# jonasBoss/ndarray-interp

Measured on AMD Instinct MI355X. Metric: interp_array Mpoints/s (queries x lanes), 1D cubic f64, higher is better.
Workload: dtype f64; 1 GPU; Target: 1D CubicSpline NotAKnot, 4096 knots x 4096 lanes f64, 10000000 queries per GPU in 4 distinct chunks of 2500000 through a 2-slot device-output ring (sorted-unique uniform knots, unsorted uniform in-range queries; output 327.7 GB per step, never copied to the host)

## Files before the change

ndarray-interp_amd/csrc/float_host.hpp:

```cpp

template <class T>
struct Queries {
  const T* a = nullptr;
  const T* b = nullptr;
  int count() const { return b ? 2 : 1; }
  Queries operator+(uint64_t off) const { return {a + off, b ? b + off : nullptr}; }
};

struct FirstFail {
  unsigned long long f0 = NO_FAIL, f1 = NO_FAIL;
  unsigned long long first() const { return std::min(f0, f1); }
  template <class T>
  static FirstFail of(const Workspace& ws, Queries<T> q) {
    return {ws.host_status->first_fail[0], q.b ? ws.host_status->first_fail[1] : NO_FAIL};
  }
};

constexpr size_t ZERO_COPY_LIMIT = 1u << 20;

template <class Plan>
struct RingRun {
  std::unique_lock<std::mutex> own;
  std::vector<void*> slots;
  uint64_t pitch = 0, chunk = 0;
  uint32_t n_slots = 0;
  uint32_t wmax = 1;
  bool narrow_first = false;
  uint32_t n_sets = 2;
  uint64_t prepped = 0;
  std::vector<Plan> plans;
  hipStream_t side = nullptr;
};

template <class T, class Impl>
struct FloatEngine {
  Impl& self() { return static_cast<Impl&>(*this); }

  ndi_status report(Queries<T> q, int q_space, FirstFail f, uint64_t index_offset, ndi_oob_info* info) {
    const int axis = f.f0 <= f.f1 ? 0 : 1;
    const unsigned long long ff = axis ? f.f1 : f.f0;
    const T* src = axis ? q.b : q.a;
    T v;
    if (q_space == NDI_MEM_DEVICE) NDI_HIP(hipMemcpy(&v, src + ff, sizeof(T), hipMemcpyDeviceToHost));
    else v = src[ff];
    const ndi_status st = self().failure_status(v);
    if (info) {
// ... 177 lines not shown
    if (out_stride < self().lanes) return fail(NDI_BAD_ARG, "out_row_stride (%llu) < lanes (%llu)",
                                               (unsigned long long)out_stride, (unsigned long long)self().lanes);
    if (nq == 0) return NDI_OK;
    if (!q_.a || q_.count() != Impl::query_arrays || !out_) return fail(NDI_BAD_ARG, "null query / output pointer");
    SpaceLease lease(self().spaces, s);
    Workspace& ws = lease.ws;
    if (self().zero_copy_fits(nq, o.q_memspace, o.out_memspace))
      return eval_small_zero_copy(s, ws, q_, nq, (T*)out_, out_stride, info);
    const Queries<T> q = stage_queries(s, ws, q_, nq, o.q_memspace);
    return eval_body(s, ws, q, q_, o.q_memspace, nq, out_, out_stride, o, info);
  }

  static constexpr bool ring_groups = false;

  template <class Plan>
  void ring_prep(hipStream_t s, Workspace& ws, Queries<T> q, uint64_t k, uint64_t cq, RingRun<Plan>& R, int path,
                 bool beside_eval) {
    Scratch& sc = ws.sc[k % R.n_sets];
    if (k >= R.n_sets) NDI_HIP(hipStreamWaitEvent(R.side, sc.eval_done, 0));
    R.plans[k % R.n_sets] = self().prep(R.side, sc, q + k * R.chunk, cq, (T*)R.slots[k % R.n_slots], R.pitch, path,
                                        beside_eval);
    NDI_HIP(hipEventRecord(sc.prep_done, R.side));
  }

  template <class Plan>
  void ring_begin(hipStream_t s, Workspace& ws, Queries<T> q, uint64_t nq, const ndi_ring_desc* ring, uint64_t stride,
                  const ndi_eval_opts& o, RingRun<Plan>& R) {
    R.n_slots = ring->n_slots;
    R.chunk = ring->chunk_queries;
    R.slots.resize(ring->n_slots);
    R.pitch = stride;
    if (ring->slots) {
      for (uint32_t i = 0; i < ring->n_slots; ++i) R.slots[i] = ring->slots[i];
    } else {
      OwnedRing& ring_own = self().ring_own;
      R.own = std::unique_lock<std::mutex>(ring_own.mu);
      ring_own.ensure(ring->n_slots, ring->chunk_queries, stride * sizeof(T));
      for (uint32_t i = 0; i < ring->n_slots; ++i) R.slots[i] = (char*)ring_own.buf.p + (size_t)i * stride * sizeof(T);
      R.pitch = (uint64_t)ring->n_slots * stride;
    }
    R.side = ring_overlap() ? ws.side_stream() : s;
    const int mode = Impl::ring_groups ? ring_group_mode() : 0;
    R.wmax = mode ? std::min<uint32_t>({R.n_slots, (uint32_t)RING_GROUP_MAX, Workspace::MAX_SETS / 2}) : 1u;
    R.narrow_first = mode == 2;
    R.n_sets = 2 * R.wmax;
    R.plans.assign(R.n_sets, Plan{});
    for (uint32_t i = 0; i < R.n_sets; ++i) ws.sc[i].ensure_events();
    NDI_HIP(hipEventRecord(ws.order_event(), s));
    NDI_HIP(hipStreamWaitEvent(R.side, ws.order_event(), 0));
    uint64_t first = 1;
    if constexpr (Impl::ring_groups)
      if (!R.narrow_first) first = std::min<uint64_t>(R.wmax, (nq + R.chunk - 1) / R.chunk);
    for (R.prepped = 0; R.prepped < first;) {
      const uint64_t k = R.prepped++;
      ring_prep(s, ws, q, k, std::min<uint64_t>(R.chunk, nq - k * R.chunk), R, o.path, false);
      if constexpr (Impl::ring_groups)
        if (!self().groupable(R.plans[k])) break;
    }
  }

  template <class Plan>
  void ring_produce(hipStream_t s, Workspace& ws, Queries<T> q, uint64_t limit, RingRun<Plan>& R,
                    ndi_ring_consumer consume, void* user, const ndi_eval_opts& o, uint64_t q_offset, uint32_t shard) {
    std::vector<hipEvent_t> busy(R.n_slots, nullptr);
    const uint64_t nchunks = (limit + R.chunk - 1) / R.chunk;
    auto count = [&](uint64_t k) { return std::min<uint64_t>(R.chunk, limit - k * R.chunk); };
    bool solo = R.wmax == 1;
    uint64_t prepped = R.prepped;
    for (uint64_t k = 0; k < nchunks;) {
      uint32_t want = solo || (R.narrow_first && k == 0) ? 1u : (uint32_t)std::min<uint64_t>(R.wmax, nchunks - k);
      uint32_t w = 0;
      while (w < want) {
        if (k + w >= prepped) {
          ring_prep(s, ws, q, k + w, count(k + w), R, o.path, R.side != s);
          prepped = k + w + 1;
        }
        bool joins = w == 0;
        if constexpr (Impl::ring_groups) joins = joins || (self().groupable(R.plans[k % R.n_sets]) &&
                                                          self().groupable(R.plans[(k + w) % R.n_sets]));
        if (!joins) break;
        ++w;
      }
      Scratch* sets[RING_GROUP_MAX];
      Plan plans[RING_GROUP_MAX];
      for (uint32_t i = 0; i < w; ++i) {
        sets[i] = &ws.sc[(k + i) % R.n_sets];
        plans[i] = R.plans[(k + i) % R.n_sets];
        NDI_HIP(hipStreamWaitEvent(s, sets[i]->prep_done, 0));
        const uint32_t slot = (uint32_t)((k + i) % R.n_slots);
// ... 9 lines not shown
          grouped = true;
        }
      if (!grouped) self().launch_eval(s, *sets[0], plans[0]);
      for (uint32_t i = 0; i < w; ++i) NDI_HIP(hipEventRecord(sets[i]->eval_done, s));
      for (uint32_t i = 0; i < w && consume; ++i) {
        const uint32_t slot = (uint32_t)((k + i) % R.n_slots);
        ndi_ring_chunk c{};
        c.index = k + i; c.q_begin = q_offset + (k + i) * R.chunk; c.q_count = count(k + i); c.out = R.slots[slot];
        c.row_stride = R.pitch; c.slot = slot; c.shard = shard; c.stream = (void*)s;
        busy[slot] = (hipEvent_t)consume(user, &c);
        if (busy[slot]) solo = true;
      }
      k += w;
    }
    NDI_HIP(hipStreamSynchronize(s));
    NDI_HIP(hipStreamSynchronize(R.side));
    for (hipEvent_t e : busy)
      if (e) NDI_HIP(hipEventSynchronize(e));
    ws.pending = false;
  }

  ndi_status run_ring(const char* range, Queries<T> q_, uint64_t nq, const ndi_ring_desc* ring, ndi_ring_consumer consume,
                      void* user, const ndi_eval_opts* opts, ndi_oob_info* info) {
    DeviceGuard dg(self().device);
    ndi_eval_opts o{};
    if (const ndi_status vs__ = take_opts(opts, o); vs__ != NDI_OK) return vs__;
    hipStream_t s = (hipStream_t)o.stream;
    uint64_t stride = 0;
    ndi_status rs = check_ring_desc(ring, self().lanes, &stride);
    if (rs != NDI_OK) return rs;
    if (nq == 0) return NDI_OK;
    if (!q_.a || q_.count() != Impl::query_arrays) return fail(NDI_BAD_ARG, "null query pointer");
    Range rg(range);
    SpaceLease lease(self().spaces, s);
    Workspace& ws = lease.ws;
    const Queries<T> q = stage_queries(s, ws, q_, nq, o.q_memspace);
    enqueue_prepass(s, ws, q, nq);
    RingRun<typename Impl::Plan> R;
    ring_begin(s, ws, q, nq, ring, stride, o, R);
    NDI_HIP(hipStreamSynchronize(s));
    const FirstFail f = FirstFail::of(ws, q);
    const uint64_t limit = f.first() == NO_FAIL ? nq : std::min<uint64_t>(nq, f.first());
    ring_produce(s, ws, q, limit, R, consume, user, o, 0, 0);
    if (f.first() == NO_FAIL) return NDI_OK;
    return report(q_, o.q_memspace, f, 0, info);
  }

  void trim_front() {
    self().spaces.trim();
    if constexpr (Impl::ring) {
      std::lock_guard<std::mutex> g(self().ring_own.mu);
// ... 5 lines not shown
```

ndarray-interp_amd/csrc/interp1d_host.hpp:

```cpp
#pragma once

template <class A, class = void>
struct takes_knots : std::false_type {};
template <class A>
struct takes_knots<A, std::void_t<decltype(std::declval<A&>().knots)>> : std::true_type {};
template <class A, class T>
static void table_args(A& F, const Interp1DImpl<T>& h) {
  if constexpr (takes_knots<A>::value) F.knots = h.pyr.view.lv0;
  else F.pyr = h.pyr.view;
  F.data = h.data.template as<T>();
  F.ca = h.ca.template as<T>();
  F.cb = h.cb.template as<T>();
}

template <class A, class T>
static void batch_args(A& F, const Interp1DImpl<T>& h, StatusBlock* st, const T* q, T* out, uint64_t nq, uint64_t out_stride) {
  F.q = q;
  F.out = out;
  F.nq = nq;
  F.out_stride = out_stride;
  F.lanes = (uint32_t)h.lanes;
  F.mode = h.mode;
  F.first_fail = &st->first_fail[0];
}
// ... 103 lines not shown
  const size_t w_plain = best_tb(false, tb_plain);
  const size_t w_lut = (P.nq >= 4096 && h.pyr.lut_bytes != 0) ? best_tb(true, tb_lut) : 0;
  if (w_plain == 0 && w_lut == 0) return false;
  P.f_lut = w_lut != 0 && 2 * w_lut >= w_plain;
  tb_auto = P.f_lut ? tb_lut : tb_plain;
  return true;
}

template <class T>
static void fused_table_form1(const Interp1DImpl<T>& h, Plan1<T>& P, const ShortKnobs& K, unsigned tb_auto) {
  const uint64_t lanes = h.lanes;
  P.f_tlds = 0;
  P.f_tb = fused_tb_or(K, tb_auto);
  if (K.lds == 0) return;
  size_t best_waves = 0;
  const bool yk_ok = h.strategy == NDI_CUBIC_SPLINE && h.ck.p;
  const int pinned = (K.lds == 2 && !yk_ok) ? 1 : K.lds;
  for (int form : {1, 2}) {
    if (form == 2 && !yk_ok) continue;
    if (pinned > 0 && pinned <= 2 && pinned != form) continue;
    for (unsigned tb : {1024u, 512u, 256u}) {
      if (K.tb && (unsigned)K.tb != tb) continue;
      const size_t need = h.fused_lds_bytes(P.f_lut, tb, form);
      if (need > FUSED_LDS_LIMIT) continue;
      const size_t waves = wgs_per_cu(need, tb) * (tb / 64);
      if (waves > best_waves) {
        best_waves = waves;
        P.f_tlds = form;
        P.f_tb = tb;
      }
    }
// ... 221 lines not shown
}

template <class T>
static Eval1Args<T> eval1_args(const Interp1DImpl<T>& h, Scratch& sc, const Plan1<T>& P) {
  Eval1Args<T> A{};
  table_args(A, h);
  A.q = P.q;
  A.idx = sc.idx.as<uint32_t>();
  A.t = sc.t.as<T>();
  A.out = P.out;
  A.lanes = h.lanes;
  A.out_stride = P.out_stride;
  A.nq = P.nq;
  A.status = sc.status.as<StatusBlock>();
  A.n_int = (uint32_t)(h.n - 1);
#ifdef NDI_BOUNDS
  if (env_int("NDI_BOUNDS_SELFTEST", 0)) A.n_int = 1;
#endif
  return A;
}

template <bool GROUP, class T, class Args>
static void launch_bucketed(Interp1DImpl<T>& h, hipStream_t s, uint64_t LV, unsigned gx, const Args& A) {
  constexpr int CQ = Interp1DImpl<T>::BUCKETED_CQ;
  const int U = LV >= 2048 ? 8 : (LV >= 1024 ? 4 : (LV >= 512 ? 2 : 1));
  const uint64_t segs = (LV + (uint64_t)BLOCK * U - 1) / ((uint64_t)BLOCK * U);
  const dim3 grid(gx, (unsigned)std::min<uint64_t>(segs, 64));
  const bool full = LV % ((uint64_t)BLOCK * U) == 0;
  pick<ST_CUBIC, ST_LINEAR>(h.strat(), [&](auto st_) {
    constexpr int ST = st_;
    pick_or<1, 8, 4, 2>(U, [&](auto u_) {
      constexpr int UU = u_;
      pick_bool(full, [&](auto full_) {
        if constexpr (GROUP) launch1<T>(s, PC_EVAL, grid, dim3(BLOCK), 0, eval_bucketed_group_kernel<T, ST, UU, CQ, true, full_>, A);
        else launch1<T>(s, PC_EVAL, grid, dim3(BLOCK), 0, eval_bucketed_kernel<T, ST, UU, CQ, true, full_>, A);
      });
    });
  });
}

template <class T>
static void launch_bucketed1(Interp1DImpl<T>& h, hipStream_t s, Scratch& sc, const Plan1<T>& P) {
  Eval1Args<T> A = eval1_args(h, sc, P);
  A.rec = sc.perm.as<uint4>();
// ... 109 lines not shown
template <class T>
void Interp1DImpl<T>::launch_eval_group(hipStream_t s, Scratch* const* sc, const Plan* P, uint32_t w) {
  if (trace_plan())
    std::fprintf(stderr, "[ndi plan] ring bucketed L=%llu lv=%llu width=%u nq=%llu\n", (unsigned long long)lanes,
                 (unsigned long long)P[0].LV, w, (unsigned long long)P[0].nq);
  if (w == 1) {
    launch_eval(s, *sc[0], P[0]);
    return;
  }
  if (w > (uint32_t)RING_GROUP_MAX) throw HipFailure{hipErrorInvalidValue, "launch_eval_group: group too wide", __LINE__};
  EvalGroupArgs<T> G{};
  table_args(G.A, *this);
  G.A.lanes = lanes;
  G.A.out_stride = P[0].out_stride;
  G.A.n_int = (uint32_t)(n - 1);
  G.width = w;
  constexpr int CQ = BUCKETED_CQ;
  uint64_t nmax = 0;
  for (uint32_t i = 0; i < w; ++i) {
    if (!groupable(P[i]) || P[i].out_stride != P[0].out_stride || P[i].LV != P[0].LV)
      throw HipFailure{hipErrorInvalidValue, "launch_eval_group: plans of one group differ", __LINE__};
    G.rec[i] = sc[i]->perm.as<uint4>();
    G.nq[i] = P[i].nq;
    G.out[i] = P[i].out;
    G.status[i] = sc[i]->status.as<StatusBlock>();
    nmax = std::max<uint64_t>(nmax, (P[i].nq + CQ - 1) / CQ);
  }
  const uint64_t per_xcd = (nmax * w + 7) / 8;
  launch_bucketed<true>(*this, s, P[0].LV, (unsigned)std::max<uint64_t>(8, std::min<uint64_t>(per_xcd * 8, 65528)), G);
}
// ... 1 lines not shown
```

ndarray-interp_amd/csrc/kernels.hpp:

```cpp
#pragma once
#include <hip/hip_runtime.h>
#include <stdint.h>

#include <type_traits>

namespace ndi {

constexpr unsigned long long NO_FAIL = ~0ull;
constexpr int BLOCK = 256;

enum ExtrapMode : int { EX_NO = 0, EX_YES = 1, EX_PERIODIC = 2 };
enum Strat : int { ST_LINEAR = 0, ST_CUBIC = 1 };

struct StatusBlock {
  unsigned long long first_fail[2];
  unsigned long long n_valid;
  unsigned long long periodic_mismatch;
  unsigned int ticket;
  unsigned int reserved;
};

#ifdef NDI_BOUNDS
__device__ unsigned long long g_ndi_bounds[4];
__device__ __forceinline__ unsigned long long ndi_bounds_fail(int code, int line, unsigned long long idx,
                                                              unsigned long long lim) {
  if (atomicAdd(&g_ndi_bounds[0], 1ull) == 0ull) {
    g_ndi_bounds[1] = ((unsigned long long)code << 32) | (unsigned)line;
// ... 622 lines not shown
template <class T>
struct Eval1Args {
  const T* knots;
  const T* data;
  const T* ca;
  const T* cb;
  const T* q;
  const uint32_t* idx;
  const T* t;
  T* out;
  uint64_t lanes, out_stride, nq;
  const StatusBlock* status;
  const uint4* rec;
  uint32_t run;
  uint32_t n_int;
};

template <class T>
__device__ __forceinline__ uint4 make_rec(uint32_t qi, uint32_t i, T s);
template <>
__device__ __forceinline__ uint4 make_rec<double>(uint32_t qi, uint32_t i, double s) {
  const unsigned long long b = __builtin_bit_cast(unsigned long long, s);
  return make_uint4(qi, i, (uint32_t)b, (uint32_t)(b >> 32));
}
template <>
__device__ __forceinline__ uint4 make_rec<float>(uint32_t qi, uint32_t i, float s) {
  return make_uint4(qi, i, __builtin_bit_cast(uint32_t, s), 0u);
}
__device__ __forceinline__ double rec_value(const uint4& r, double) {
  return __builtin_bit_cast(double, ((unsigned long long)r.w << 32) | r.z);
// ... 18 lines not shown
    c.c0 = x2 - x1;
    c.c1 = xq - x1;
    c.c2 = T(0);
  }
  return c;
}

template <class T, int STRAT, class V>
__device__ __forceinline__ V row_point(const RowCoef<T, STRAT>& c, V yl, V yr, V a, V b) {
  if (STRAT == ST_CUBIC) {
    return c.c0 * yl + c.c1 * yr + c.c2 * (a * c.c0 + b * c.c1);
  } else {
    V m = (yr - yl) / c.c0;
    return m * c.c1 + yl;
  }
}

template <bool NT, class V>
__device__ __forceinline__ void store_stream(V* p, V v) {
  if (NT) __builtin_nontemporal_store(v, p);
  else *p = v;
}

constexpr int SMALL_LANES = 16;

template <class T>
struct EvalSmallArgs {
  Pyramid<T> pyr;
  const T* data;
  const T* ca;
// ... 1223 lines not shown
  for (uint32_t i = threadIdx.x; i < nb; i += BLOCK) cur[i] = off[i] + base[i];
  __syncthreads();
  const uint64_t q_begin = (uint64_t)blockIdx.x * slice;
  uint64_t q_end = q_begin + slice;
  if (q_end > nq) q_end = nq;
  for (uint64_t qi = q_begin + threadIdx.x; qi < q_end; qi += BLOCK) {
    const uint32_t i = NDI_CHK(idx[qi], nb, BC_BIN);
    const uint32_t pos = NDI_CHK(atomicAdd(&cur[i], 1u), nq, BC_POSITION);
    rec[pos] = make_rec<T>((uint32_t)qi, i, sval[qi]);
  }
}

template <class T, int STRAT, int U, int CQ, bool NT = true, bool FULL = false>
__global__ __launch_bounds__(BLOCK) void eval_bucketed_kernel(Eval1Args<T> A) {
  constexpr int VN = Wide<T>::N;
  using V = typename VecT<T, VN>::type;
  __shared__ uint32_t s_q[CQ];
  __shared__ uint32_t s_i[CQ];
  __shared__ T s_s[CQ];
  const uint64_t LV = A.lanes / VN;
  const uint32_t seg_vecs = BLOCK * U;
  const uint32_t segs = (uint32_t)((LV + seg_vecs - 1) / seg_vecs);
  const unsigned long long n_valid = A.nq;
  unsigned long long limit = A.status->first_fail[0];
  if (limit > A.nq) limit = A.nq;
  const uint64_t nchunks = (n_valid + CQ - 1) / CQ;
  const uint64_t per = (nchunks + 7) / 8;
  const uint64_t run = A.run ? A.run : 1;
  const uint64_t runs_per_xcd = (per + run - 1) / run;
  for (uint32_t seg = blockIdx.y; seg < segs; seg += gridDim.y) {
// ... 6 lines not shown
      if (c_end > nchunks) c_end = nchunks;
      V ryl[U], ryr[U], ra[U], rb[U];
      uint32_t cur = 0xffffffffu;
      for (uint64_t chunk = c_begin; chunk < c_end; ++chunk) {
        const uint64_t p0 = chunk * CQ;
        const uint32_t cnt = (n_valid - p0 < (uint64_t)CQ) ? (uint32_t)(n_valid - p0) : (uint32_t)CQ;
        __syncthreads();
        for (uint32_t j = threadIdx.x; j < cnt; j += BLOCK) {
          const uint4 r = A.rec[p0 + j];
          s_q[j] = r.x;
          s_i[j] = r.y;
          s_s[j] = rec_value(r, T(0));
        }
        __syncthreads();
        auto emit = [&](uint32_t i, uint32_t qi, T sj) {
          const RowCoef<T, STRAT> c = row_coef<T, STRAT>(A.knots, i, sj, sj);
          V* o = reinterpret_cast<V*>(A.out + (uint64_t)qi * A.out_stride);
#pragma unroll
          for (int u = 0; u < U; ++u) {
            const uint64_t v = v0 + (uint64_t)u * BLOCK;
            if (FULL || v < LV) store_stream<NT>(o + v, row_point<T, STRAT, V>(c, ryl[u], ryr[u], ra[u], rb[u]));
          }
        };
        for (uint32_t j = 0; j < cnt;) {
          const uint32_t i = NDI_CHK((uint32_t)__builtin_amdgcn_readfirstlane((int)s_i[j]), A.n_int, BC_INTERVAL);
          const uint32_t qi = NDI_CHK((uint32_t)__builtin_amdgcn_readfirstlane((int)s_q[j]), A.nq, BC_QUERY);
          if (qi >= limit) { ++j; continue; }
          if (i != cur) {
            cur = i;
            const V* yl = reinterpret_cast<const V*>(A.data + (uint64_t)i * A.lanes);
            const V* yr = yl + LV;
            const V* pa = reinterpret_cast<const V*>(A.ca + (uint64_t)i * A.lanes);
            const V* pb = reinterpret_cast<const V*>(A.cb + (uint64_t)i * A.lanes);
#pragma unroll
            for (int u = 0; u < U; ++u) {
              const uint64_t v = v0 + (uint64_t)u * BLOCK;
              if (FULL || v < LV) {
                ryl[u] = yl[v];
                ryr[u] = yr[v];
                if (STRAT == ST_CUBIC) {
                  ra[u] = pa[v];
                  rb[u] = pb[v];
                }
              }
            }
          }
          emit(i, qi, s_s[j]);
          ++j;
        }
      }
    }
  }
}

constexpr int RING_GROUP_MAX = 4;
template <class T>
struct EvalGroupArgs {
  Eval1Args<T> A;
  const uint4* rec[RING_GROUP_MAX];
  uint64_t nq[RING_GROUP_MAX];
  T* out[RING_GROUP_MAX];
  const StatusBlock* status[RING_GROUP_MAX];
  uint32_t width;
};

template <class T, int STRAT, int U, int CQ, bool NT = true, bool FULL = false>
__global__ __launch_bounds__(BLOCK) void eval_bucketed_group_kernel(EvalGroupArgs<T> G) {
  constexpr int VN = Wide<T>::N;
  using V = typename VecT<T, VN>::type;
  __shared__ uint32_t s_q[CQ];
  __shared__ uint32_t s_i[CQ];
  __shared__ T s_s[CQ];
  const Eval1Args<T>& A = G.A;
  const uint64_t LV = A.lanes / VN;
  const uint32_t seg_vecs = BLOCK * U;
  const uint32_t segs = (uint32_t)((LV + seg_vecs - 1) / seg_vecs);
  const uint32_t width = G.width;
  uint64_t nmax = 0;
#pragma unroll
  for (int w = 0; w < RING_GROUP_MAX; ++w) {
    const uint64_t n_w = (uint32_t)w < width ? (G.nq[w] + CQ - 1) / CQ : 0;
    if (n_w > nmax) nmax = n_w;
  }
// ... 29 lines not shown
      unsigned long long limit = status->first_fail[0];
      if (limit > nq) limit = nq;
      V ryl[U], ryr[U], ra[U], rb[U];
      uint32_t cur = 0xffffffffu;
      const uint64_t p0 = chunk * CQ;
      const uint32_t cnt = (n_valid - p0 < (uint64_t)CQ) ? (uint32_t)(n_valid - p0) : (uint32_t)CQ;
      __syncthreads();
      for (uint32_t j = threadIdx.x; j < cnt; j += BLOCK) {
        const uint4 r = rec[p0 + j];
        s_q[j] = r.x;
        s_i[j] = r.y;
        s_s[j] = rec_value(r, T(0));
      }
      __syncthreads();
      auto emit = [&](uint32_t i, uint32_t qi, T sj) {
        const RowCoef<T, STRAT> cf = row_coef<T, STRAT>(A.knots, i, sj, sj);
        V* o = reinterpret_cast<V*>(out + (uint64_t)qi * A.out_stride);
#pragma unroll
        for (int u = 0; u < U; ++u) {
          const uint64_t v = v0 + (uint64_t)u * BLOCK;
          if (FULL || v < LV) store_stream<NT>(o + v, row_point<T, STRAT, V>(cf, ryl[u], ryr[u], ra[u], rb[u]));
        }
      };
      for (uint32_t j = 0; j < cnt;) {
        const uint32_t i = NDI_CHK((uint32_t)__builtin_amdgcn_readfirstlane((int)s_i[j]), A.n_int, BC_INTERVAL);
        const uint32_t qi = NDI_CHK((uint32_t)__builtin_amdgcn_readfirstlane((int)s_q[j]), nq, BC_QUERY);
        if (qi >= limit) { ++j; continue; }
        if (i != cur) {
          cur = i;
          const V* yl = reinterpret_cast<const V*>(A.data + (uint64_t)i * A.lanes);
          const V* yr = yl + LV;
          const V* pa = reinterpret_cast<const V*>(A.ca + (uint64_t)i * A.lanes);
          const V* pb = reinterpret_cast<const V*>(A.cb + (uint64_t)i * A.lanes);
#pragma unroll
          for (int u = 0; u < U; ++u) {
            const uint64_t v = v0 + (uint64_t)u * BLOCK;
            if (FULL || v < LV) {
              ryl[u] = yl[v];
              ryr[u] = yr[v];
              if (STRAT == ST_CUBIC) {
                ra[u] = pa[v];
                rb[u] = pb[v];
              }
            }
          }
        }
        emit(i, qi, s_s[j]);
        ++j;
      }
    }
  }
}

template <class T, int STRAT, int G, int CQ, bool NT = true>
__global__ __launch_bounds__(BLOCK) void eval_bucketed_short_kernel(Eval1Args<T> A) {
  constexpr int VN = Wide<T>::N;
  using V = typename VecT<T, VN>::type;
// ... 1885 lines not shown
      if (b < cnt) {
        const uint64_t i = hi - 1 - b;
        const T k = (ri[b] - upc[b] * k_next) / midc[b];
        const T dy = y_hi - yl[b];
        sa[i * L] = k * dxc[b] - dy;
        sb[i * L] = dy - k_next * dxc[b];
        if (KOUT) A.kout[i * L + l] = k;
        k_next = k;
        y_hi = yl[b];
      }
    }
    hi -= (uint64_t)cnt;
  }
}

template <class T, int RW>
__global__ __launch_bounds__(256) void spline_build_wide_kernel(BuildArgs<T> A) {
  extern __shared__ __attribute__((aligned(16))) unsigned char smem_raw[];
  constexpr int RB = 3 * RW;
  T* const s_r = reinterpret_cast<T*>(smem_raw);
  T* const s_y = s_r + 2 * RB * 64;
  T* const s_f = s_y + 2 * RB * 64;
  const uint32_t tid = threadIdx.x, lane = tid & 63u;
  const uint32_t wave = __builtin_amdgcn_readfirstlane(tid >> 6);
  const uint64_t n = A.n, L = A.lanes;
  const uint64_t l0 = (uint64_t)blockIdx.x * 64u, l = l0 + lane;
  const bool live = l < L;
  const uint64_t lc = live ? l : L - 1u;
  const T* __restrict__ const y = A.data;
  T* const sa = A.ca;
  T* const sb = A.cb;
// ... 92 lines not shown
      const uint64_t i = b < hi ? hi - 1 - b : 0;
      T* const f = s_f + (size_t)buf * 4 * RB;
      const SharedDivisor<T> sd = shared_divisor<T>(A.midp[i]);
      f[0 * RB + b] = A.up[i];
      f[1 * RB + b] = sd.d;
      f[2 * RB + b] = sd.ok ? sd.r : T(0);
      f[3 * RB + b] = A.dx[i];
    }
  };
  T k_next = T(0), y_hi = T(0);
  if (wave == 0) {
    const T rhs_last = spline_rhs_at<T, false, false>(A, n - 1, lc);
    const T r_last = rhs_last - A.w[n - 1] * r_prev;
    k_next = r_last / A.midp[n - 1];
    y_hi = y[(n - 1) * L + lc];
  } else {
    produce_bwd(0u, n - 1);
  }
  __syncthreads();
  auto back_row = [&](uint64_t i, T ri, T yl, T up, T mid, T rmid, T dxi) {
    SharedDivisor<T> sd;
    sd.d = mid; sd.r = rmid; sd.ok = rmid > T(0);
    const T num = ri - up * k_next;
    bool ok;
    T k = div_shared_fast<T>(num, sd, ok);
    if (__builtin_expect(!ok, 0)) k = num / mid;
    const T dy = y_hi - yl;
    if (live) {
      sa[i * L + l] = k * dxi - dy;
      sb[i * L + l] = dy - k_next * dxi;
    }
    k_next = k;
    y_hi = yl;
  };
  for (uint64_t blk = 0; blk < bblk; ++blk) {
    const uint64_t hi = n - 1 - blk * RB;
    const uint32_t buf = (uint32_t)(blk & 1u);
    if (wave != 0) {
      if (blk + 1 < bblk) produce_bwd(buf ^ 1u, hi - RB);
    } else {
      const T* const r = s_r + (size_t)buf * RB * 64;
      const T* const yy = s_y + (size_t)buf * RB * 64;
      const T* const f = s_f + (size_t)buf * 4 * RB;
      if (hi >= (uint64_t)RB) {
#pragma unroll
// ... 426 lines not shown
```

ndarray-interp_amd/csrc/ndinterp_api.hip:

```cpp
#include <dlfcn.h>

#include <algorithm>
#include <atomic>
#include <chrono>
#include <condition_variable>
#include <cmath>
#include <cstdlib>
#include <cstring>
#include <functional>
#include <limits>
#include <map>
#include <memory>
#include <mutex>
#include <set>
#include <shared_mutex>
#include <stdexcept>
#include <thread>
#include <unordered_map>
#include <utility>
#include <vector>

#include "common.hpp"
#include "host_logic.hpp"
#include "kernels.hpp"
// ... 411 lines not shown
  }
  void ensure_events() {
    if (!prep_done) NDI_HIP(hipEventCreateWithFlags(&prep_done, hipEventDisableTiming));
    if (!eval_done) NDI_HIP(hipEventCreateWithFlags(&eval_done, hipEventDisableTiming));
  }
};

struct Workspace {
  static constexpr uint32_t MAX_SETS = 8;
  Scratch sc[MAX_SETS];
  DevBuf status, qdev, qdev2, stage;
  StatusBlock* host_status = nullptr;
  void* pin = nullptr;
  void* pin_dev = nullptr;
  size_t pin_bytes = 0;
  hipStream_t side = nullptr;
  hipEvent_t ev = nullptr;
  uint64_t last_nq = 0;
  const void* last_q = nullptr;
  const void* last_q2 = nullptr;
  int last_q_space = NDI_MEM_DEVICE;
  bool pending = false;
  int users = 0;
  uint64_t last_use = 0;
  ~Workspace() {
    if (side) (void)hipStreamDestroy(side);
    if (ev) (void)hipEventDestroy(ev);
    if (host_status) (void)hipHostFree(host_status);
    if (pin) (void)hipHostFree(pin);
  }
  void ensure_pin(size_t need) {
    if (need <= pin_bytes) return;
    if (pin) (void)hipHostFree(pin);
    pin = nullptr;
    pin_dev = nullptr;
    pin_bytes = 0;
    NDI_HIP(hipHostMalloc(&pin, need, hipHostMallocMapped | hipHostMallocPortable));
    NDI_HIP(hipHostGetDevicePointer(&pin_dev, pin, 0));
    pin_bytes = need;
  }
  template <class U>
  U* pin_device(const void* host_ptr) const {
    return reinterpret_cast<U*>((char*)pin_dev + ((const char*)host_ptr - (const char*)pin));
  }
  void ensure_status() {
    status.reserve(sizeof(StatusBlock));
    for (int i = 0; i < 2; ++i) sc[i].status.reserve(sizeof(StatusBlock));
    if (!host_status) NDI_HIP(hipHostMalloc((void**)&host_status, sizeof(StatusBlock), hipHostMallocDefault));
  }
  hipStream_t side_stream() {
    if (!side) {
      int lo = 0, hi = 0;
      NDI_HIP(hipDeviceGetStreamPriorityRange(&lo, &hi));
      NDI_HIP(hipStreamCreateWithPriority(&side, hipStreamNonBlocking, hi));
    }
    return side;
  }
  hipEvent_t order_event() {
    if (!ev) NDI_HIP(hipEventCreateWithFlags(&ev, hipEventDisableTiming));
    return ev;
  }
};

struct SpaceSet {
  static constexpr size_t MAX_IDLE = 16;
  std::mutex mu;
  std::map<SpaceKey, std::unique_ptr<Workspace>> map;
  uint64_t tick = 0;

  Workspace& acquire(hipStream_t s) {
    std::lock_guard<std::mutex> g(mu);
// ... 418 lines not shown
      packed_state.store(1, std::memory_order_release);
      return true;
    }
    (void)hipGetLastError();
    if (s != packed_stream) NDI_HIP(hipStreamWaitEvent(s, packed_ev, 0));
    return true;
  }

  void adopt_arena(bool cubic, bool with_k) {
    auto al = [](size_t b) { return (b + 255) & ~(size_t)255; };
    uint64_t block = 1;
    while ((uint64_t)64 * block < n) block *= 2;
    const size_t pyr_b = al((n + (n + block - 1) / block) * sizeof(T));
    const size_t data_b = al((size_t)n * lanes * sizeof(T));
    const size_t tab_b = cubic ? al((size_t)(n - 1) * lanes * sizeof(T)) : 0;
    const size_t k_b = (cubic && with_k && 2 * data_b <= FUSED_LDS_LIMIT) ? data_b : 0;
    const size_t total = pyr_b + data_b + 2 * tab_b + k_b;
    if (total > ((size_t)1 << 20)) return;
    arena.reserve(total);
    char* p0 = static_cast<char*>(arena.p);
    pyr.buf.adopt(p0, pyr_b);
    data.adopt(p0 + pyr_b, data_b);
    if (tab_b) {
      ca.adopt(p0 + pyr_b + data_b, tab_b);
      cb.adopt(p0 + pyr_b + data_b + tab_b, tab_b);
    }
    if (k_b) ck.adopt(p0 + pyr_b + data_b + 2 * tab_b, k_b);
  }

  uint64_t signature() const override {
    uint64_t h = fnv1a(FNV_SEED, pyr.host_knots.data(), pyr.host_knots.size() * sizeof(T));
    const uint64_t f[3] = {n, (uint64_t)strategy | ((uint64_t)rule << 8) | ((uint64_t)deriv << 16), (uint64_t)mode};
    return fnv1a(h, f, sizeof(f));
  }

  T* reserve_k() {
    static const Knob keep{"NDI_SPLINE_KEEP_K", 1, Knob::live};
    if (!keep.get() || lanes > 2048 || fused_lds_bytes(false, 256, 2) > FUSED_LDS_LIMIT) {
      ck.release();
      return nullptr;
    }
    ck.reserve((size_t)n * lanes * sizeof(T));
    return ck.as<T>();
  }

  ndi_status build_spline(const ndi_interp1d_desc& d);
  ndi_status build_hermite(const void* dydx, int memspace);

  using Plan = Plan1<T>;
  Plan prep(hipStream_t s, Scratch& sc, const T* q, uint64_t nq, T* out, uint64_t out_stride, int path,
            bool beside_eval = false, int flags = 0);
  void launch_eval(hipStream_t s, Scratch& sc, const Plan& P);

// ... 1054 lines not shown
  uint64_t lo, cnt;
  DeviceGuard dg;
  hipStream_t s;
  SpaceLease lease;
  Workspace& ws;
  Queries<T> q_src, q;
  uint64_t stride = 0;
  RingRun<typename Impl::Plan> R;
  Shard(const Job<Impl>& j, uint32_t i_, uint32_t n)
      : J(j), i(i_), h(j.H[i_]), lo(shard_lo(j.nq, i_, n)), cnt(shard_lo(j.nq, i_ + 1, n) - shard_lo(j.nq, i_, n)),
        dg(h->device), s((hipStream_t)(j.io ? j.io[i_].stream : nullptr)), lease(h->spaces, s), ws(lease.ws),
        q_src(j.q_src(i_, n)) {}
  void pre(unsigned long long* fx, unsigned long long* fy) {
    if (!cnt) return;
    q = h->stage_queries(s, ws, q_src, cnt, J.o.q_memspace);
    h->enqueue_prepass(s, ws, q, cnt);
    if (J.rings) {
      (void)check_ring_desc(&J.rings[i], h->lanes, &stride);
      h->ring_begin(s, ws, q, cnt, &J.rings[i], stride, J.o, R);
    }
    NDI_HIP(hipStreamSynchronize(s));
    const FirstFail f = FirstFail::of(ws, q);
    *fx = f.f0;
    *fy = f.f1;
  }
  ndi_status run(uint64_t limit) {
    if (!cnt) return NDI_OK;
    if (J.rings) {
      h->ring_produce(s, ws, q, limit, R, J.consume, J.user, J.o, lo, i);
      return NDI_OK;
// ... 1102 lines not shown
```

ndarray-interp_amd/csrc/spline_build_host.hpp:

```cpp
#pragma once

template <class T>
static void reserve_tables(Interp1DImpl<T>& h) {
  const size_t tab = (size_t)(h.n - 1) * h.lanes * sizeof(T);
  h.ca.reserve(tab);
  h.cb.reserve(tab);
}

static unsigned build_rows_grid(uint64_t n, uint64_t lanes) {
  return (unsigned)std::max<uint64_t>(1, std::min<uint64_t>((n * lanes + BLOCK - 1) / BLOCK, 65536));
}
static unsigned build_lane_grid(uint64_t lanes) { return (unsigned)((lanes + 63) / 64); }

template <class T>
static BuildArgs<T> build_args(Interp1DImpl<T>& h, const SplinePlan<T>& P) {
  BuildArgs<T> A{};
  A.data = h.data.template as<T>();
  A.ca = h.ca.template as<T>();
  A.cb = h.cb.template as<T>();
  A.n = h.n;
  A.lanes = h.lanes;
  A.left_kind = P.left_kind;
  A.right_kind = P.right_kind;
  A.left_val = P.left_val;
// ... 183 lines not shown
  }
  NDI_HIP(hipGetLastError());
  if (per) NDI_HIP(hipMemcpy(&hs, tmp.p, sizeof(hs), hipMemcpyDeviceToHost));
  else NDI_HIP(hipStreamSynchronize(s));
}

template <class T>
static void build_serial(int spline_mode, const BuildArgs<T>& A, const BuildTemp<T>& tmp, StatusBlock& hs) {
  const uint64_t n = A.n, lanes = A.lanes;
  const unsigned grid = build_lane_grid(lanes);
  hipStream_t s = nullptr;
  switch (spline_mode) {
    case SPLINE_GENERAL: {
      static const Knob wide_knob{"NDI_SPLINE_WIDE", -1, Knob::live};
      const int wide_env = wide_knob.get();
      if (!A.kout && n >= 4 && (wide_env > 0 || (wide_env < 0 && lanes >= 1024))) {
        constexpr int RW = 16, RBW = 3 * RW;
        const size_t shm = (size_t)(4 * RBW * 64 + 2 * 4 * RBW) * sizeof(T);
        auto kern = spline_build_wide_kernel<T, RW>;
        allow_dynamic_lds(reinterpret_cast<const void*>(kern), (int)shm);
        hipLaunchKernelGGL(kern, dim3(grid), dim3(256), shm, s, A);
        break;
      }
      hipLaunchKernelGGL((spline_rhs_kernel<T, false>), dim3(build_rows_grid(n, lanes)), dim3(BLOCK), 0, s, A);
      launch_build_general<T, false, false>(A);
      break;
    }
    case SPLINE_PARABOLA3:
      hipLaunchKernelGGL(spline_build_n3_kernel<T>, dim3(grid), dim3(64), 0, s, A, 0);
      break;
    case SPLINE_PERIODIC3:
      hipLaunchKernelGGL(spline_build_n3_kernel<T>, dim3(grid), dim3(64), 0, s, A, 1);
      break;
    case SPLINE_PERIODIC:
      hipLaunchKernelGGL(spline_build_periodic_kernel<T>, dim3(grid), dim3(64), 0, s, A);
      break;
// ... 154 lines not shown
```

Before: 863,200 Mpoints/s.

## Use knot-slope table in bucketed cubic eval and split ring prep across side streams

```diff
diff --git a/ndarray-interp_amd/csrc/float_host.hpp b/ndarray-interp_amd/csrc/float_host.hpp
--- a/ndarray-interp_amd/csrc/float_host.hpp
+++ b/ndarray-interp_amd/csrc/float_host.hpp
@@ -30,6 +30,8 @@
   uint64_t prepped = 0;
   std::vector<Plan> plans;
   hipStream_t side = nullptr;
+  hipStream_t sides[Workspace::MAX_SIDES] = {};
+  uint32_t n_sides = 1;
 };
 
 template <class T, class Impl>
@@ -237,14 +239,16 @@
   static constexpr bool ring_groups = false;
 
   template <class Plan>
-  void ring_prep(hipStream_t s, Workspace& ws, Queries<T> q, uint64_t k, uint64_t cq, RingRun<Plan>& R, int path,
+  void ring_prep(hipStream_t side, Workspace& ws, Queries<T> q, uint64_t k, uint64_t cq, RingRun<Plan>& R, int path,
                  bool beside_eval) {
     Scratch& sc = ws.sc[k % R.n_sets];
-    if (k >= R.n_sets) NDI_HIP(hipStreamWaitEvent(R.side, sc.eval_done, 0));
-    R.plans[k % R.n_sets] = self().prep(R.side, sc, q + k * R.chunk, cq, (T*)R.slots[k % R.n_slots], R.pitch, path,
+    if (k >= R.n_sets) NDI_HIP(hipStreamWaitEvent(side, sc.eval_done, 0));
+    R.plans[k % R.n_sets] = self().prep(side, sc, q + k * R.chunk, cq, (T*)R.slots[k % R.n_slots], R.pitch, path,
                                         beside_eval);
-    NDI_HIP(hipEventRecord(sc.prep_done, R.side));
-  }
+    NDI_HIP(hipEventRecord(sc.prep_done, side));
+  }
+
+  void ring_order(hipStream_t s, Workspace& ws) { NDI_HIP(hipEventRecord(ws.order_event(), s)); }
 
   template <class Plan>
   void ring_begin(hipStream_t s, Workspace& ws, Queries<T> q, uint64_t nq, const ndi_ring_desc* ring, uint64_t stride,
@@ -262,21 +266,27 @@
       for (uint32_t i = 0; i < ring->n_slots; ++i) R.slots[i] = (char*)ring_own.buf.p + (size_t)i * stride * sizeof(T);
       R.pitch = (uint64_t)ring->n_slots * stride;
     }
-    R.side = ring_overlap() ? ws.side_stream() : s;
+    R.side = R.sides[0] = ring_overlap() ? ws.side_stream(0) : s;
+    R.n_sides = 1;
     const int mode = Impl::ring_groups ? ring_group_mode() : 0;
     R.wmax = mode ? std::min<uint32_t>({R.n_slots, (uint32_t)RING_GROUP_MAX, Workspace::MAX_SETS / 2}) : 1u;
     R.narrow_first = mode == 2;
     R.n_sets = 2 * R.wmax;
     R.plans.assign(R.n_sets, Plan{});
     for (uint32_t i = 0; i < R.n_sets; ++i) ws.sc[i].ensure_events();
-    NDI_HIP(hipEventRecord(ws.order_event(), s));
-    NDI_HIP(hipStreamWaitEvent(R.side, ws.order_event(), 0));
     uint64_t first = 1;
     if constexpr (Impl::ring_groups)
       if (!R.narrow_first) first = std::min<uint64_t>(R.wmax, (nq + R.chunk - 1) / R.chunk);
+    if (ring_overlap())
+      while (R.n_sides < std::min<uint64_t>(first, Workspace::MAX_SIDES)) {
+        R.sides[R.n_sides] = ws.side_stream(R.n_sides);
+        ++R.n_sides;
+      }
+    for (uint32_t j = 0; j < R.n_sides; ++j)
+      if (R.sides[j] != s) NDI_HIP(hipStreamWaitEvent(R.sides[j], ws.order_event(), 0));
     for (R.prepped = 0; R.prepped < first;) {
       const uint64_t k = R.prepped++;
-      ring_prep(s, ws, q, k, std::min<uint64_t>(R.chunk, nq - k * R.chunk), R, o.path, false);
+      ring_prep(R.sides[k % R.n_sides], ws, q, k, std::min<uint64_t>(R.chunk, nq - k * R.chunk), R, o.path, false);
       if constexpr (Impl::ring_groups)
         if (!self().groupable(R.plans[k])) break;
     }
@@ -295,7 +305,7 @@
       uint32_t w = 0;
       while (w < want) {
         if (k + w >= prepped) {
-          ring_prep(s, ws, q, k + w, count(k + w), R, o.path, R.side != s);
+          ring_prep(R.side, ws, q, k + w, count(k + w), R, o.path, R.side != s);
           prepped = k + w + 1;
         }
         bool joins = w == 0;
@@ -335,7 +345,7 @@
       k += w;
     }
     NDI_HIP(hipStreamSynchronize(s));
-    NDI_HIP(hipStreamSynchronize(R.side));
+    for (uint32_t j = 0; j < R.n_sides; ++j) NDI_HIP(hipStreamSynchronize(R.sides[j]));
     for (hipEvent_t e : busy)
       if (e) NDI_HIP(hipEventSynchronize(e));
     ws.pending = false;
@@ -356,6 +366,7 @@
     SpaceLease lease(self().spaces, s);
     Workspace& ws = lease.ws;
     const Queries<T> q = stage_queries(s, ws, q_, nq, o.q_memspace);
+    ring_order(s, ws);
     enqueue_prepass(s, ws, q, nq);
     RingRun<typename Impl::Plan> R;
     ring_begin(s, ws, q, nq, ring, stride, o, R);
diff --git a/ndarray-interp_amd/csrc/interp1d_host.hpp b/ndarray-interp_amd/csrc/interp1d_host.hpp
--- a/ndarray-interp_amd/csrc/interp1d_host.hpp
+++ b/ndarray-interp_amd/csrc/interp1d_host.hpp
@@ -141,7 +141,7 @@
   P.f_tb = fused_tb_or(K, tb_auto);
   if (K.lds == 0) return;
   size_t best_waves = 0;
-  const bool yk_ok = h.strategy == NDI_CUBIC_SPLINE && h.ck.p;
+  const bool yk_ok = h.strategy == NDI_CUBIC_SPLINE && h.ck.p && h.k_fits_lds();
   const int pinned = (K.lds == 2 && !yk_ok) ? 1 : K.lds;
   for (int form : {1, 2}) {
     if (form == 2 && !yk_ok) continue;
@@ -393,11 +393,15 @@
   A.nq = P.nq;
   A.status = sc.status.as<StatusBlock>();
   A.n_int = (uint32_t)(h.n - 1);
+  A.ck = h.ck.template as<T>();
 #ifdef NDI_BOUNDS
   if (env_int("NDI_BOUNDS_SELFTEST", 0)) A.n_int = 1;
 #endif
   return A;
 }
+
+template <class T>
+static bool bucketed_k_rows(const Interp1DImpl<T>& h) { return h.ck.p != nullptr && h.k_for_long_rows(); }
 
 template <bool GROUP, class T, class Args>
 static void launch_bucketed(Interp1DImpl<T>& h, hipStream_t s, uint64_t LV, unsigned gx, const Args& A) {
@@ -406,7 +410,9 @@
   const uint64_t segs = (LV + (uint64_t)BLOCK * U - 1) / ((uint64_t)BLOCK * U);
   const dim3 grid(gx, (unsigned)std::min<uint64_t>(segs, 64));
   const bool full = LV % ((uint64_t)BLOCK * U) == 0;
-  pick<ST_CUBIC, ST_LINEAR>(h.strat(), [&](auto st_) {
+  if (trace_plan() && h.strategy == NDI_CUBIC_SPLINE)
+    std::fprintf(stderr, "[ndi rows] bucketed tables=%s u=%d full=%d\n", bucketed_k_rows(h) ? "{y,k}" : "{y,a,b}", U, (int)full);
+  pick<ST_CUBIC, ST_LINEAR, ST_CUBIC_K>(bucketed_k_rows(h) ? (int)ST_CUBIC_K : h.strat(), [&](auto st_) {
     constexpr int ST = st_;
     pick_or<1, 8, 4, 2>(U, [&](auto u_) {
       constexpr int UU = u_;
@@ -546,6 +552,7 @@
   G.A.lanes = lanes;
   G.A.out_stride = P[0].out_stride;
   G.A.n_int = (uint32_t)(n - 1);
+  G.A.ck = ck.template as<T>();
   G.width = w;
   constexpr int CQ = BUCKETED_CQ;
   uint64_t nmax = 0;
diff --git a/ndarray-interp_amd/csrc/kernels.hpp b/ndarray-interp_amd/csrc/kernels.hpp
--- a/ndarray-interp_amd/csrc/kernels.hpp
+++ b/ndarray-interp_amd/csrc/kernels.hpp
@@ -10,7 +10,8 @@
 constexpr int BLOCK = 256;
 
 enum ExtrapMode : int { EX_NO = 0, EX_YES = 1, EX_PERIODIC = 2 };
-enum Strat : int { ST_LINEAR = 0, ST_CUBIC = 1 };
+enum Strat : int { ST_LINEAR = 0, ST_CUBIC = 1, ST_CUBIC_K = 2 };
+constexpr int poly_strat(int strat) { return strat == ST_CUBIC_K ? (int)ST_CUBIC : strat; }
 
 struct StatusBlock {
   unsigned long long first_fail[2];
@@ -663,6 +664,7 @@
   const uint4* rec;
   uint32_t run;
   uint32_t n_int;
+  const T* ck;
 };
 
 template <class T>
@@ -711,6 +713,19 @@
     V m = (yr - yl) / c.c0;
     return m * c.c1 + yl;
   }
+}
+
+constexpr int vmcnt_imm(int n) { return (n & 15) | ((n >> 4) << 14) | (7 << 4) | (15 << 8); }
+__device__ __forceinline__ void wait_vmcnt(int n) {
+#define NDI_VMCNT(N) case N: __builtin_amdgcn_s_waitcnt(vmcnt_imm(N)); break;
+  switch (n) {
+    NDI_VMCNT(0) NDI_VMCNT(1) NDI_VMCNT(2) NDI_VMCNT(3) NDI_VMCNT(4) NDI_VMCNT(5) NDI_VMCNT(6) NDI_VMCNT(7)
+    NDI_VMCNT(8) NDI_VMCNT(9) NDI_VMCNT(10) NDI_VMCNT(11) NDI_VMCNT(12) NDI_VMCNT(13) NDI_VMCNT(14) NDI_VMCNT(15)
+    NDI_VMCNT(16) NDI_VMCNT(17) NDI_VMCNT(18) NDI_VMCNT(19) NDI_VMCNT(20) NDI_VMCNT(21) NDI_VMCNT(22) NDI_VMCNT(23)
+    NDI_VMCNT(24) NDI_VMCNT(25) NDI_VMCNT(26) NDI_VMCNT(27) NDI_VMCNT(28) NDI_VMCNT(29) NDI_VMCNT(30) NDI_VMCNT(31)
+    default: break;
+  }
+#undef NDI_VMCNT
 }
 
 template <bool NT, class V>
@@ -1964,6 +1979,7 @@
 template <class T, int STRAT, int U, int CQ, bool NT = true, bool FULL = false>
 __global__ __launch_bounds__(BLOCK) void eval_bucketed_kernel(Eval1Args<T> A) {
   constexpr int VN = Wide<T>::N;
+  constexpr int PS = poly_strat(STRAT);
   using V = typename VecT<T, VN>::type;
   __shared__ uint32_t s_q[CQ];
   __shared__ uint32_t s_i[CQ];
@@ -2000,12 +2016,13 @@
         }
         __syncthreads();
         auto emit = [&](uint32_t i, uint32_t qi, T sj) {
-          const RowCoef<T, STRAT> c = row_coef<T, STRAT>(A.knots, i, sj, sj);
+          const RowCoef<T, PS> c = row_coef<T, PS>(A.knots, i, sj, sj);
           V* o = reinterpret_cast<V*>(A.out + (uint64_t)qi * A.out_stride);
 #pragma unroll
           for (int u = 0; u < U; ++u) {
             const uint64_t v = v0 + (uint64_t)u * BLOCK;
-            if (FULL || v < LV) store_stream<NT>(o + v, row_point<T, STRAT, V>(c, ryl[u], ryr[u], ra[u], rb[u]));
+            if (STRAT == ST_CUBIC_K) wait_vmcnt(4 * U - 4 - 3 * u);
+            if (FULL || v < LV) store_stream<NT>(o + v, row_point<T, PS, V>(c, ryl[u], ryr[u], ra[u], rb[u]));
           }
         };
         for (uint32_t j = 0; j < cnt;) {
@@ -2016,17 +2033,29 @@
             cur = i;
             const V* yl = reinterpret_cast<const V*>(A.data + (uint64_t)i * A.lanes);
             const V* yr = yl + LV;
-            const V* pa = reinterpret_cast<const V*>(A.ca + (uint64_t)i * A.lanes);
-            const V* pb = reinterpret_cast<const V*>(A.cb + (uint64_t)i * A.lanes);
+            const V* pa = reinterpret_cast<const V*>((STRAT == ST_CUBIC_K ? A.ck : A.ca) + (uint64_t)i * A.lanes);
+            const V* pb = STRAT == ST_CUBIC_K ? pa + LV : reinterpret_cast<const V*>(A.cb + (uint64_t)i * A.lanes);
 #pragma unroll
             for (int u = 0; u < U; ++u) {
               const uint64_t v = v0 + (uint64_t)u * BLOCK;
               if (FULL || v < LV) {
                 ryl[u] = yl[v];
                 ryr[u] = yr[v];
-                if (STRAT == ST_CUBIC) {
+                if (STRAT != ST_LINEAR) {
                   ra[u] = pa[v];
                   rb[u] = pb[v];
+                }
+              }
+            }
+            if (STRAT == ST_CUBIC_K) {
+              const T dx = A.knots[i + 1] - A.knots[i];
+#pragma unroll
+              for (int u = 0; u < U; ++u) {
+                const uint64_t v = v0 + (uint64_t)u * BLOCK;
+                if (FULL || v < LV) {
+                  const V dy = ryr[u] - ryl[u];
+                  ra[u] = ra[u] * dx - dy;
+                  rb[u] = dy - rb[u] * dx;
                 }
               }
             }
@@ -2053,6 +2082,7 @@
 template <class T, int STRAT, int U, int CQ, bool NT = true, bool FULL = false>
 __global__ __launch_bounds__(BLOCK) void eval_bucketed_group_kernel(EvalGroupArgs<T> G) {
   constexpr int VN = Wide<T>::N;
+  constexpr int PS = poly_strat(STRAT);
   using V = typename VecT<T, VN>::type;
   __shared__ uint32_t s_q[CQ];
   __shared__ uint32_t s_i[CQ];
@@ -2112,12 +2142,13 @@
       }
       __syncthreads();
       auto emit = [&](uint32_t i, uint32_t qi, T sj) {
-        const RowCoef<T, STRAT> cf = row_coef<T, STRAT>(A.knots, i, sj, sj);
+        const RowCoef<T, PS> cf = row_coef<T, PS>(A.knots, i, sj, sj);
         V* o = reinterpret_cast<V*>(out + (uint64_t)qi * A.out_stride);
 #pragma unroll
         for (int u = 0; u < U; ++u) {
           const uint64_t v = v0 + (uint64_t)u * BLOCK;
-          if (FULL || v < LV) store_stream<NT>(o + v, row_point<T, STRAT, V>(cf, ryl[u], ryr[u], ra[u], rb[u]));
+          if (STRAT == ST_CUBIC_K) wait_vmcnt(4 * U - 4 - 3 * u);
+          if (FULL || v < LV) store_stream<NT>(o + v, row_point<T, PS, V>(cf, ryl[u], ryr[u], ra[u], rb[u]));
         }
       };
       for (uint32_t j = 0; j < cnt;) {
@@ -2128,17 +2159,29 @@
           cur = i;
           const V* yl = reinterpret_cast<const V*>(A.data + (uint64_t)i * A.lanes);
           const V* yr = yl + LV;
-          const V* pa = reinterpret_cast<const V*>(A.ca + (uint64_t)i * A.lanes);
-          const V* pb = reinterpret_cast<const V*>(A.cb + (uint64_t)i * A.lanes);
+          const V* pa = reinterpret_cast<const V*>((STRAT == ST_CUBIC_K ? A.ck : A.ca) + (uint64_t)i * A.lanes);
+          const V* pb = STRAT == ST_CUBIC_K ? pa + LV : reinterpret_cast<const V*>(A.cb + (uint64_t)i * A.lanes);
 #pragma unroll
           for (int u = 0; u < U; ++u) {
             const uint64_t v = v0 + (uint64_t)u * BLOCK;
             if (FULL || v < LV) {
               ryl[u] = yl[v];
               ryr[u] = yr[v];
-              if (STRAT == ST_CUBIC) {
+              if (STRAT != ST_LINEAR) {
                 ra[u] = pa[v];
                 rb[u] = pb[v];
+              }
+            }
+          }
+          if (STRAT == ST_CUBIC_K) {
+            const T dx = A.knots[i + 1] - A.knots[i];
+#pragma unroll
+            for (int u = 0; u < U; ++u) {
+              const uint64_t v = v0 + (uint64_t)u * BLOCK;
+              if (FULL || v < LV) {
+                const V dy = ryr[u] - ryl[u];
+                ra[u] = ra[u] * dx - dy;
+                rb[u] = dy - rb[u] * dx;
               }
             }
           }
@@ -4054,7 +4097,7 @@
   }
 }
 
-template <class T, int RW>
+template <class T, int RW, bool KOUT = false>
 __global__ __launch_bounds__(256) void spline_build_wide_kernel(BuildArgs<T> A) {
   extern __shared__ __attribute__((aligned(16))) unsigned char smem_raw[];
   constexpr int RB = 3 * RW;
@@ -4177,6 +4220,7 @@
     const T r_last = rhs_last - A.w[n - 1] * r_prev;
     k_next = r_last / A.midp[n - 1];
     y_hi = y[(n - 1) * L + lc];
+    if (KOUT && live) A.kout[(n - 1) * L + l] = k_next;
   } else {
     produce_bwd(0u, n - 1);
   }
@@ -4192,6 +4236,7 @@
     if (live) {
       sa[i * L + l] = k * dxi - dy;
       sb[i * L + l] = dy - k_next * dxi;
+      if (KOUT) A.kout[i * L + l] = k;
     }
     k_next = k;
     y_hi = yl;
diff --git a/ndarray-interp_amd/csrc/ndinterp_api.hip b/ndarray-interp_amd/csrc/ndinterp_api.hip
--- a/ndarray-interp_amd/csrc/ndinterp_api.hip
+++ b/ndarray-interp_amd/csrc/ndinterp_api.hip
@@ -449,7 +449,8 @@
   void* pin = nullptr;
   void* pin_dev = nullptr;
   size_t pin_bytes = 0;
-  hipStream_t side = nullptr;
+  static constexpr uint32_t MAX_SIDES = 2;
+  hipStream_t side[MAX_SIDES] = {};
   hipEvent_t ev = nullptr;
   uint64_t last_nq = 0;
   const void* last_q = nullptr;
@@ -459,7 +460,8 @@
   int users = 0;
   uint64_t last_use = 0;
   ~Workspace() {
-    if (side) (void)hipStreamDestroy(side);
+    for (hipStream_t sd : side)
+      if (sd) (void)hipStreamDestroy(sd);
     if (ev) (void)hipEventDestroy(ev);
     if (host_status) (void)hipHostFree(host_status);
     if (pin) (void)hipHostFree(pin);
@@ -483,13 +485,13 @@
     for (int i = 0; i < 2; ++i) sc[i].status.reserve(sizeof(StatusBlock));
     if (!host_status) NDI_HIP(hipHostMalloc((void**)&host_status, sizeof(StatusBlock), hipHostMallocDefault));
   }
-  hipStream_t side_stream() {
-    if (!side) {
+  hipStream_t side_stream(uint32_t j) {
+    if (!side[j]) {
       int lo = 0, hi = 0;
       NDI_HIP(hipDeviceGetStreamPriorityRange(&lo, &hi));
-      NDI_HIP(hipStreamCreateWithPriority(&side, hipStreamNonBlocking, hi));
-    }
-    return side;
+      NDI_HIP(hipStreamCreateWithPriority(&side[j], hipStreamNonBlocking, hi));
+    }
+    return side[j];
   }
   hipEvent_t order_event() {
     if (!ev) NDI_HIP(hipEventCreateWithFlags(&ev, hipEventDisableTiming));
@@ -938,7 +940,7 @@
     const size_t pyr_b = al((n + (n + block - 1) / block) * sizeof(T));
     const size_t data_b = al((size_t)n * lanes * sizeof(T));
     const size_t tab_b = cubic ? al((size_t)(n - 1) * lanes * sizeof(T)) : 0;
-    const size_t k_b = (cubic && with_k && 2 * data_b <= FUSED_LDS_LIMIT) ? data_b : 0;
+    const size_t k_b = (cubic && with_k && (2 * data_b <= FUSED_LDS_LIMIT || k_for_long_rows())) ? data_b : 0;
     const size_t total = pyr_b + data_b + 2 * tab_b + k_b;
     if (total > ((size_t)1 << 20)) return;
     arena.reserve(total);
@@ -958,9 +960,14 @@
     return fnv1a(h, f, sizeof(f));
   }
 
+  bool k_fits_lds() const { return lanes <= 2048 && fused_lds_bytes(false, 256, 2) <= FUSED_LDS_LIMIT; }
+  bool k_for_long_rows() const {
+    return strategy == NDI_CUBIC_SPLINE && rule == HR_SPLINE && deriv == 0 && lanes % Wide<T>::N == 0 &&
+           lanes / Wide<T>::N >= (uint64_t)BLOCK;
+  }
   T* reserve_k() {
     static const Knob keep{"NDI_SPLINE_KEEP_K", 1, Knob::live};
-    if (!keep.get() || lanes > 2048 || fused_lds_bytes(false, 256, 2) > FUSED_LDS_LIMIT) {
+    if (!keep.get() || !(k_fits_lds() || k_for_long_rows())) {
       ck.release();
       return nullptr;
     }
@@ -2045,6 +2052,7 @@
   void pre(unsigned long long* fx, unsigned long long* fy) {
     if (!cnt) return;
     q = h->stage_queries(s, ws, q_src, cnt, J.o.q_memspace);
+    if (J.rings) h->ring_order(s, ws);
     h->enqueue_prepass(s, ws, q, cnt);
     if (J.rings) {
       (void)check_ring_desc(&J.rings[i], h->lanes, &stride);
diff --git a/ndarray-interp_amd/csrc/spline_build_host.hpp b/ndarray-interp_amd/csrc/spline_build_host.hpp
--- a/ndarray-interp_amd/csrc/spline_build_host.hpp
+++ b/ndarray-interp_amd/csrc/spline_build_host.hpp
@@ -221,12 +221,14 @@
     case SPLINE_GENERAL: {
       static const Knob wide_knob{"NDI_SPLINE_WIDE", -1, Knob::live};
       const int wide_env = wide_knob.get();
-      if (!A.kout && n >= 4 && (wide_env > 0 || (wide_env < 0 && lanes >= 1024))) {
+      if (n >= 4 && (wide_env > 0 || (wide_env < 0 && lanes >= 1024))) {
         constexpr int RW = 16, RBW = 3 * RW;
         const size_t shm = (size_t)(4 * RBW * 64 + 2 * 4 * RBW) * sizeof(T);
-        auto kern = spline_build_wide_kernel<T, RW>;
-        allow_dynamic_lds(reinterpret_cast<const void*>(kern), (int)shm);
-        hipLaunchKernelGGL(kern, dim3(grid), dim3(256), shm, s, A);
+        pick_bool(A.kout != nullptr, [&](auto kout_) {
+          auto kern = spline_build_wide_kernel<T, RW, kout_>;
+          allow_dynamic_lds(reinterpret_cast<const void*>(kern), (int)shm);
+          hipLaunchKernelGGL(kern, dim3(grid), dim3(256), shm, s, A);
+        });
         break;
       }
       hipLaunchKernelGGL((spline_rhs_kernel<T, false>), dim3(build_rows_grid(n, lanes)), dim3(BLOCK), 0, s, A);
```

After: 871,400 Mpoints/s (median of 6 runs). About the same (+0.9%).
